# LargeWorldModel/LWM

Hardware: AMD Instinct MI355X
Metric: tokens/sec fwd+bwd, LWM-7B RingAttention hot path (32 layers x 32 heads x 128) (higher is better)
Workload: dtype bf16 (f32 logits/softmax/accumulate)

## Files before the change

lwm_amd/csrc/attn_bwd64.h:

```cpp
#pragma once

namespace lwm {

constexpr int kD4BK = 128;
constexpr int kD4BQ = 64;
constexpr int kD4Threads = 256;
constexpr int kD4Slots = 4;
constexpr int kD4TileBytes = kD4BQ * kRowBytes;
constexpr int kD4SlotBytes = 2 * kD4TileBytes;
constexpr int kD4OffStat = kD4Slots * kD4SlotBytes;
constexpr int kD4StatBytes = 3 * kD4BQ * 4;
constexpr int kD4LdsBytes = kD4OffStat + kD4Slots * kD4StatBytes;
#ifndef LWM_D4_AHEAD
#define LWM_D4_AHEAD 6
#endif
constexpr int kD4Ahead = LWM_D4_AHEAD;
static_assert(kD4Ahead >= 1 && kD4Ahead <= 7, "prefetch distance in fragments");
static_assert((kD4Ahead % 2) == 0, "paired requests need an even distance");

constexpr int q4_swz_of(int row) {
    const int r = row & 15;
    return (((r & 7) << 1) | (r >> 3)) ^ ((r >= 4 && r < 12) ? 1 : 0);
}
LWM_DEVICE int q4_swz(int row) { return q4_swz_of(row); }
LWM_DEVICE uint32_t q4_tile_off(int row, int slot) { return (uint32_t)(row * kRowBytes + ((slot ^ q4_swz(row)) << 4)); }
constexpr bool q4_image_ok() {
    for (int s = 0; s < 4; ++s)
        for (int grp = 0; grp < 4; ++grp) {
            unsigned long long banks = 0;
            for (int l = 0; l < 64; ++l) {
                const int m = l & 31;
                const bool first = m < 4 || (m >= 12 && m < 16) || (m >= 20 && m < 28);
                if (2 * (l >> 5) + (first ? 0 : 1) != grp) continue;
                const int slot = (4 * s + (l >> 4)) ^ q4_swz_of(l & 15);
                const unsigned long long b = 0xFull << (4 * slot);
                if (banks & b) return false;
                banks |= b;
            }
            if (banks != ~0ull) return false;
        }
    for (int db = 0; db < 8; ++db)
        for (int up = 0; up < 2; ++up)
            for (int half = 0; half < 2; ++half) {
                unsigned long long banks = 0;
                for (int l = 32 * half; l < 32 * half + 32; ++l) {
                    const int g = l >> 4, t = l & 15, row = 16 * up + 4 * g + (t >> 2);
                    const int slot = (2 * db + ((t & 3) >> 1)) ^ q4_swz_of(row);
                    const unsigned long long b = 0x3ull << (4 * slot + 2 * (t & 1));
                    if (banks & b) return false;
                    banks |= b;
                }
                if (banks != ~0ull) return false;
            }
    return true;
}
static_assert(q4_image_ok(), "a read of the Q | dO (K | V) image is bank-conflicted");

#ifdef LWM_EMU
LWM_DEVICE f32x4 mfma_16x16x32(bf16x8 a, bf16x8 b, f32x4 c) {
    emu::Wave& w = emu::g_blk->waves[emu::g_lane->tid >> 6];
    const int l = emu::g_lane->tid & 63;
    w.a[l] = a;
    w.b[l] = b;
    emu::wave_sync();
    f32x4 d;
    const int col = l & 15, g = l >> 4;
    for (int j = 0; j < 4; ++j) {
        const int row = 4 * g + j;
        float s = c[j];
        for (int k = 0; k < 32; ++k) s += (float)w.a[(k >> 3) * 16 + row][k & 7] * (float)w.b[(k >> 3) * 16 + col][k & 7];
        d[j] = s;
    }
    emu::wave_sync();
    return d;
}
LWM_DEVICE void q4_mfma_first(f32x4& d, bf16x8 a, bf16x8 b) { d = mfma_16x16x32(a, b, f32x4{0.0f, 0.0f, 0.0f, 0.0f}); }
LWM_DEVICE void q4_mfma(f32x4& d, bf16x8 a, bf16x8 b) { d = mfma_16x16x32(a, b, d); }
LWM_DEVICE void q4_mfma_c_first(f32x4& d, bf16x8 a, bf16x8 b, const f32x4& c) { d = mfma_16x16x32(a, b, c); }
LWM_DEVICE void q4_mfma_o(f32x4& d, bf16x8 a, bf16x8 b) { d = mfma_16x16x32(a, b, d); }
LWM_DEVICE void q4_mfma_o_first(f32x4& d, bf16x8 a, bf16x8 b) { d = mfma_16x16x32(a, b, f32x4{0.0f, 0.0f, 0.0f, 0.0f}); }
LWM_DEVICE void q4_opaque(f32x4 (&)[2]) {}
LWM_DEVICE void q4_settle_t(f32x4 (&)[4]) {}
LWM_DEVICE void q4_settle_acc(f32x4 (&)[16]) {}
#else
LWM_DEVICE void q4_mfma_first(f32x4& d, bf16x8 a, bf16x8 b) {
    asm volatile("v_mfma_f32_16x16x32_bf16 %0, %1, %2, 0" : "=&v"(d) : "v"(a), "a"(b));
}
LWM_DEVICE void q4_mfma(f32x4& d, bf16x8 a, bf16x8 b) {
    asm volatile("v_mfma_f32_16x16x32_bf16 %0, %1, %2, %0" : "+v"(d) : "v"(a), "a"(b));
}
LWM_DEVICE void q4_mfma_c_first(f32x4& d, bf16x8 a, bf16x8 b, const f32x4& c) {
    asm volatile("s_nop 1\n\tv_mfma_f32_16x16x32_bf16 %0, %1, %2, %3" : "=&v"(d) : "v"(a), "a"(b), "v"(c));
}
LWM_DEVICE void q4_mfma_o(f32x4& d, bf16x8 a, bf16x8 b) {
    asm volatile("v_mfma_f32_16x16x32_bf16 %0, %1, %2, %0" : "+a"(d) : "v"(a), "v"(b));
}
LWM_DEVICE void q4_mfma_o_first(f32x4& d, bf16x8 a, bf16x8 b) {
    asm volatile("v_mfma_f32_16x16x32_bf16 %0, %1, %2, 0" : "=&a"(d) : "v"(a), "v"(b));
}
LWM_DEVICE void q4_opaque(f32x4 (&x)[2]) { asm volatile("" : "+v"(x[0]), "+v"(x[1])); }
LWM_DEVICE void q4_settle_t(f32x4 (&s)[4]) { asm volatile("s_nop 7\n\ts_nop 7" : "+v"(s[0]), "+v"(s[1]), "+v"(s[2]), "+v"(s[3])); }
LWM_DEVICE void q4_settle_acc(f32x4 (&a)[16]) {
    asm volatile("s_nop 7\n\ts_nop 7"
                 : "+a"(a[0]), "+a"(a[1]), "+a"(a[2]), "+a"(a[3]), "+a"(a[4]), "+a"(a[5]), "+a"(a[6]), "+a"(a[7]), "+a"(a[8]),
                   "+a"(a[9]), "+a"(a[10]), "+a"(a[11]), "+a"(a[12]), "+a"(a[13]), "+a"(a[14]), "+a"(a[15]));
}
#endif

constexpr int kDsTileBytes = kD4BQ * 32 * 2;
constexpr int64_t ds_diag(int causal, int64_t q_start, int64_t k_start) {
    const int64_t lim = (int64_t)1 << 30, e = (k_start - q_start) >> 6;
    return !causal ? -lim : (e < -lim ? -lim : (e > lim ? lim : e));
}
constexpr int64_t ds_first_step(int64_t e, int64_t nst, int64_t kbi) {
    const int64_t s = e + 2 * kbi;
    return s < 0 ? 0 : (s > nst ? nst : s);
}
constexpr int64_t ds_steps_before(int64_t e, int64_t nst, int64_t kbi) {
    const int64_t jl = e >= 0 ? 0 : (1 - e) >> 1;
    const int64_t jh0 = e >= nst ? 0 : (nst - e + 1) >> 1;
    const int64_t jh = jh0 > jl ? jh0 : jl;
    const int64_t a = kbi < jl ? kbi : jl, b = kbi < jh ? kbi : jh;
    return kbi * nst - ((b - a) * e + (b - a) * (a + b - 1) + (kbi - b) * nst);
}
constexpr bool ds_geom_ok() {
    const int64_t es[] = {-(1 << 30), -1000, -9, -8, -3, -2, -1, 0, 1, 2, 3, 7, 8, 9, 40, 1 << 30};
    const int64_t ns[] = {1, 2, 3, 4, 6, 8, 9, 32};
    for (int64_t e : es)
        for (int64_t nst : ns) {
            int64_t sum = 0;
            for (int64_t kbi = 0; kbi < 24; ++kbi) {
                if (ds_steps_before(e, nst, kbi) != sum) return false;
                sum += nst - ds_first_step(e, nst, kbi);
            }
        }
    return true;
}
static_assert(ds_geom_ok(), "closed form of the workspace row offsets disagrees with the sum it stands for");
constexpr int64_t ds_wave_steps(int64_t e, int64_t nst, int64_t nkb, int64_t s) {
    if (s >= nst) return 0;
    const int64_t kend = s - e < 0 ? 0 : ((s - e) >> 1) + 1;
    return 4 * (kend < nkb ? kend : nkb);
}
constexpr int64_t ds_ws_bytes(int64_t B, int64_t H, int64_t Sq, int64_t Sk, int causal, int64_t q_start, int64_t k_start) {
    return B * H * ds_steps_before(ds_diag(causal, q_start, k_start), Sq / kD4BQ, Sk / kD4BK) * 4 * kDsTileBytes;
}

struct D4Ds {
    char* p;
    uint32_t v;
};
#ifdef LWM_EMU
LWM_DEVICE char* ds_uniform_ptr(char* p) { return p; }
template <int OFF>
LWM_DEVICE void d4_ds_store(const D4Ds& sw, bf16x8 x) { memcpy(sw.p + OFF + sw.v, &x, 16); }
#else
LWM_DEVICE char* ds_uniform_ptr(char* p) {
    const uint64_t a = (uint64_t)p;
    return (char*)(((uint64_t)(uint32_t)__builtin_amdgcn_readfirstlane((int)(a >> 32)) << 32) | (uint32_t)__builtin_amdgcn_readfirstlane((int)a));
}
template <int OFF>
LWM_DEVICE void d4_ds_store(const D4Ds& sw, bf16x8 x) {
    static_assert(OFF >= -4096 && OFF <= 4095, "13-bit signed instruction offset");
    asm volatile("global_store_dwordx4 %0, %1, %2 offset:%3 nt" ::"v"(sw.v), "v"(x), "s"(sw.p), "n"(OFF) : "memory");
}
#endif

struct D4Ctx {
    uint32_t qa[4];
    uint32_t tlo[8];
    uint32_t plo[8];
    uint32_t stat;
    float c;
};

#ifdef LWM_EMU
LWM_DEVICE float d4_mul(float a, float b) { return a * b; }
LWM_DEVICE void d4_dma_b32(uint32_t voff, const char* src, lds_t dst) { glds_load_b32(src + voff, dst); }
LWM_DEVICE void d4_settle_acc4(f32x16 (&)[4]) {}
#else
LWM_DEVICE float d4_mul(float a, float b) {
    float y;
    asm volatile("v_mul_f32 %0, %1, %2" : "=v"(y) : "v"(a), "v"(b));
    return y;
}
LWM_DEVICE void d4_dma_b32(uint32_t voff, const char* src, lds_t dst) {
    const uint64_t a = (uint64_t)src;
    const uint64_t u = ((uint64_t)(uint32_t)__builtin_amdgcn_readfirstlane((int)(a >> 32)) << 32) |
                       (uint32_t)__builtin_amdgcn_readfirstlane((int)a);
    asm volatile("s_mov_b32 m0, %2\n\ts_nop 0\n\tglobal_load_lds_dword %0, %1" ::"v"(voff), "s"(u), "s"(dst) : "memory");
}
LWM_DEVICE void d4_settle_acc4(f32x16 (&a)[4]) { asm volatile("s_nop 7\n\ts_nop 7" : "+a"(a[0]), "+a"(a[1]), "+a"(a[2]), "+a"(a[3])); }
#endif
LWM_DEVICE void d4_mfma_p_first(f32x4& d, bf16x8 a, bf16x8 b, const f32x4& c) { q4_mfma_c_first(d, a, b, c); }
LWM_DEVICE void d4_mfma_o_first(f32x4& d, bf16x8 a, bf16x8 b) { q4_mfma_o_first(d, a, b); }
LWM_DEVICE void d4_settle_t(f32x4 (&s)[4]) { q4_settle_t(s); }
LWM_DEVICE void d4_settle_acc(f32x4 (&dk)[16], f32x4 (&dv)[16]) {
    q4_settle_acc(dk);
    q4_settle_acc(dv);
}

LWM_DEVICE void d4_stage_offsets(const AttnParams& p, int wave, int lane, int st, uint32_t (&vq)[4], uint32_t (&vdo)[4]) {
    const int slot = lane & 15;
    for (int j = 0; j < 4; ++j) {
        const int row = 4 * (wave + 4 * j) + (lane >> 4);
        int qrow = st * kD4BQ + row;
        qrow = qrow < p.Sq ? qrow : p.Sq - 1;
        const int rel = qrow - st * kD4BQ;
        const int col = (slot ^ q4_swz(row)) << 3;
        vq[j] = (uint32_t)(((int64_t)rel * p.q_ss + col) * 2);
        vdo[j] = (uint32_t)(((int64_t)rel * p.do_ss + col) * 2);
    }
}

template <int HALF>
LWM_DEVICE bf16x8 d4_frag(const D4Ctx& cx, int f) {
    if (f >= 32) {
        const int g = f - 32;
        return lds_read_b128(cx.qa[g >> 2] + ((g >> 1) & 1) * kD4TileBytes + (g & 1) * 16 * kRowBytes + (HALF == 0 ? 32 * kRowBytes : 0));
    }
    if (f < 16) return lds_read_b128(cx.qa[f >> 2] + ((f >> 1) & 1) * kD4TileBytes + (f & 1) * 16 * kRowBytes + HALF * 32 * kRowBytes);
    const int j = f - 16, db = 2 * (j >> 2) + (j & 1);
    const uint32_t a = (HALF == 0 ? cx.plo[db] : cx.tlo[db]) + (HALF == 0 ? 32 * kRowBytes : 0) + (((j >> 1) & 1) ? 0 : kD4TileBytes);
    bf16x4 lo = lds_read_tr16(a);
    bf16x4 up = lds_read_tr16(a + 16 * kRowBytes);
    bf16x8 o;
    o[0] = lo[0]; o[1] = lo[1]; o[2] = lo[2]; o[3] = lo[3];
    o[4] = up[0]; o[5] = up[1]; o[6] = up[2]; o[7] = up[3];
    return o;
}

struct D4Sched {
    int F[16], E[16], M[16], P[8], D[8], W[2];
};
constexpr bool d4_sched_ok(const D4Sched& c) {
    int load[64] = {};
    for (int e = 0; e < 16; ++e) {
        if (c.F[e] < 3 || c.F[e] > 31 || c.E[e] <= c.F[e] || c.M[e] <= c.E[e] || c.M[e] > 61) return false;
        load[c.F[e]] += 1;
        load[c.E[e]] += 2;
        load[c.M[e]] += 1;
    }
    for (int i = 0; i < 8; ++i) {
        if (c.P[i] < 32 || c.P[i] > 61 || c.P[i] <= c.E[2 * i] || c.P[i] <= c.E[2 * i + 1]) return false;
        if (c.D[i] < 32 || c.D[i] > 61 || c.D[i] <= c.M[2 * i] || c.D[i] <= c.M[2 * i + 1]) return false;
        load[c.P[i]] += 1;
        load[c.D[i]] += 1;
    }
    for (int h = 0; h < 2; ++h) {
        if (c.W[h] != 63) return false;
        for (int i = 4 * h; i < 4 * h + 4; ++i)
            if (c.W[h] <= c.D[i]) return false;
    }
    for (int g = 0; g < 64; ++g)
        if (load[g] > 2) return false;
    return true;
}
constexpr D4Sched kD4Sched = {
     {3, 3, 4, 4, 5, 5, 6, 6, 7, 7, 8, 8, 9, 9, 10, 10},
     {11, 12, 13, 14, 15, 16, 17, 18, 19, 20, 21, 22, 23, 24, 25, 26},
     {27, 27, 28, 28, 29, 29, 30, 30, 31, 31, 32, 32, 33, 33, 34, 34},
     {35, 35, 36, 36, 37, 37, 38, 38},
     {39, 39, 40, 40, 41, 41, 42, 42},
     {63, 63}};
static_assert(d4_sched_ok(kD4Sched), "filler schedule violates a dependency or the issue budget of a gap");

struct D4Dma {
    const char* q_src;
    const char* do_src;
    lds_t dst;
};

struct D4Regs {
    f32x4 s[4];
    f32x4 dp[2][4];
    f32x4 ndl[2];
    float nl[8];
    float t[16];
    float ds[16];
    bf16x8 pb[2], dsb[2];
    uint32_t pw[8], dw[8];
    bf16x8 fr[8];
};

template <int G, int PAR>
LWM_DEVICE void d4_fillers(const D4Ctx& cx, D4Regs& rg) {
#pragma unroll
    for (int e = 0; e < 16; ++e) {
        if (kD4Sched.F[e] == G) rg.t[e] = f4_fma(rg.s[e >> 2][e & 3], cx.c, rg.nl[4 * ((e >> 2) & 1) + (e & 3)]);
        if (kD4Sched.E[e] == G) rg.t[e] = f4_exp2(rg.t[e]);
        if (kD4Sched.M[e] == G) rg.ds[e] = d4_mul(rg.t[e], rg.dp[PAR][e >> 2][e & 3]);
    }
#pragma unroll
    for (int i = 0; i < 8; ++i) {
        if (kD4Sched.P[i] == G) rg.pw[i] = f4_cvt_pk(rg.t[2 * i], rg.t[2 * i + 1]);
        if (kD4Sched.D[i] == G) rg.dw[i] = f4_cvt_pk(rg.ds[2 * i], rg.ds[2 * i + 1]);
    }
#pragma unroll
    for (int h = 0; h < 2; ++h) {
        int lp = 0, ld = 0;
        for (int i = 4 * h; i < 4 * h + 4; ++i) {
            lp = kD4Sched.P[i] > lp ? kD4Sched.P[i] : lp;
            ld = kD4Sched.D[i] > ld ? kD4Sched.D[i] : ld;
        }
        if (lp == G) rg.pb[h] = __builtin_bit_cast(bf16x8, u32x4{rg.pw[4 * h], rg.pw[4 * h + 1], rg.pw[4 * h + 2], rg.pw[4 * h + 3]});
        if (ld == G) rg.dsb[h] = __builtin_bit_cast(bf16x8, u32x4{rg.dw[4 * h], rg.dw[4 * h + 1], rg.dw[4 * h + 2], rg.dw[4 * h + 3]});
    }
}

template <int G, int BASE>
LWM_DEVICE void d4_ds_stores(const D4Ds& sw, const D4Regs& rg) {
    if constexpr (kD4Sched.W[0] == G) d4_ds_store<BASE>(sw, rg.dsb[0]);
    if constexpr (kD4Sched.W[1] == G) d4_ds_store<BASE + 1024>(sw, rg.dsb[1]);
}

template <int HALF, bool HAS_PREV, bool DMA, bool DS, int M = 0>
LWM_DEVICE void d4_x(const D4Ctx& cx, D4Regs& rg, const bf16x8 (&kf)[8], const bf16x8 (&vf)[8], const uint32_t (&vq)[4],
                     const uint32_t (&vdo)[4], const D4Dma& dm, const D4Ds& sw) {
    if constexpr (M < 32) {
        if constexpr ((M & 3) == 0) {
            constexpr int f0 = (M >> 1) + kD4Ahead;
            rg.fr[f0 & 7] = d4_frag<HALF>(cx, f0);
            sched_fence();
            rg.fr[(f0 + 1) & 7] = d4_frag<HALF>(cx, f0 + 1);
        }
        if constexpr (M == 10 || M == 18) {
            constexpr int qh = M == 18 ? 1 : 0;
            const f32x4 v = lds_read_f32x4(cx.stat + (HALF * 32 + 16 * qh) * 4);
            rg.nl[4 * qh + 0] = v[0]; rg.nl[4 * qh + 1] = v[1]; rg.nl[4 * qh + 2] = v[2]; rg.nl[4 * qh + 3] = v[3];
        }
        sched_fence();
        {
            constexpr int f = (M >> 1) ^ 1, qh = f & 1, kh = ((M >> 1) ^ M) & 1;
            constexpr int s = f >> 2, t = 2 * kh + qh;
            if constexpr (((f >> 1) & 1) == 0) {
                if constexpr (s == 0) q4_mfma_first(rg.s[t], rg.fr[f & 7], kf[4 * kh]);
                else q4_mfma(rg.s[t], rg.fr[f & 7], kf[4 * kh + s]);
            } else {
                if constexpr (s == 0) d4_mfma_p_first(rg.dp[HALF][t], rg.fr[f & 7], vf[4 * kh], rg.ndl[qh]);
                else q4_mfma(rg.dp[HALF][t], rg.fr[f & 7], vf[4 * kh + s]);
            }
        }
        if constexpr (DMA && (M & 3) == 3) {
            constexpr int i = M >> 2, j = i >> 1;
            if constexpr ((i & 1) == 0) f4_dma1(vq[j], dm.q_src, dm.dst + 4096 * j);
            else f4_dma1(vdo[j], dm.do_src, dm.dst + kD4TileBytes + 4096 * j);
        }
        if constexpr (HAS_PREV) d4_fillers<32 + M, HALF ^ 1>(cx, rg);
        if constexpr (HAS_PREV && DS) d4_ds_stores<32 + M, HALF == 1 ? -kDsTileBytes : kDsTileBytes / 2>(sw, rg);
        sched_fence();
        d4_x<HALF, HAS_PREV, DMA, DS, M + 1>(cx, rg, kf, vf, vq, vdo, dm, sw);
    }
}

template <int HALF, bool HAS_META>
LWM_DEVICE void d4_mask(const D4Ctx& cx, f32x4 (&s)[4], const int (&rel)[2], const int32_t (&kseg)[2]) {
#pragma unroll
    for (int qh = 0; qh < 2; ++qh) {
        u32x4 sg = {0u, 0u, 0u, 0u};
        if (HAS_META) sg = lds_read_u32x4(cx.stat + 2 * kD4BQ * 4 + HALF * 32 * 4 + 16 * qh * 4);
#pragma unroll
        for (int kh = 0; kh < 2; ++kh)
#pragma unroll
            for (int j = 0; j < 4; ++j) {
                const bool vis = (!HAS_META || (int32_t)sg[j] == kseg[kh]) && (16 * qh + j >= rel[kh]);
                s[2 * kh + qh][j] = vis ? s[2 * kh + qh][j] : -INFINITY;
            }
    }
}

template <int HALF, bool HAS_PREV, bool NEXT, bool INIT, int J = 0>
LWM_DEVICE void d4_y(const D4Ctx& cx, D4Regs& rg, f32x4 (&dk)[16], f32x4 (&dv)[16], uint32_t statn) {
    if constexpr (J < 32) {
        if constexpr ((J & 3) == 0 && (16 + (J >> 1) + kD4Ahead < 32 || NEXT)) {
            constexpr int f0 = 16 + (J >> 1) + kD4Ahead;
            rg.fr[f0 & 7] = d4_frag<HALF>(cx, f0);
            sched_fence();
            rg.fr[(f0 + 1) & 7] = d4_frag<HALF>(cx, f0 + 1);
        }
        if constexpr (NEXT && (J == 22 || J == 26)) {
            constexpr int qh = J == 26 ? 1 : 0;
            rg.ndl[qh] = lds_read_f32x4(statn + kD4BQ * 4 + ((HALF ^ 1) * 32 + 16 * qh) * 4);
        }
        sched_fence();
        if constexpr (HAS_PREV) {
            constexpr int jf = (J >> 1) ^ 1, kh = ((J >> 1) ^ J) & 1;
            constexpr int db = 2 * (jf >> 2) + (jf & 1);
            if constexpr (((jf >> 1) & 1) == 0) {
                if constexpr (INIT) d4_mfma_o_first(dv[2 * db + kh], rg.fr[(16 + jf) & 7], rg.pb[kh]);
                else q4_mfma_o(dv[2 * db + kh], rg.fr[(16 + jf) & 7], rg.pb[kh]);
            } else {
                if constexpr (INIT) d4_mfma_o_first(dk[2 * db + kh], rg.fr[(16 + jf) & 7], rg.dsb[kh]);
                else q4_mfma_o(dk[2 * db + kh], rg.fr[(16 + jf) & 7], rg.dsb[kh]);
            }
        }
        d4_fillers<J, HALF>(cx, rg);
        sched_fence();
        d4_y<HALF, HAS_PREV, NEXT, INIT, J + 1>(cx, rg, dk, dv, statn);
    }
}

template <int PAR, bool DS, int G = 32>
LWM_DEVICE void d4_drain_fill(const D4Ctx& cx, D4Regs& rg, const D4Ds& sw) {
    if constexpr (G < 64) {
        d4_fillers<G, PAR>(cx, rg);
        if constexpr (DS) d4_ds_stores<G, kDsTileBytes / 2>(sw, rg);
        d4_drain_fill<PAR, DS, G + 1>(cx, rg, sw);
    }
}
template <int H, int J = 0>
LWM_DEVICE void d4_drain_mfma(D4Regs& rg, f32x4 (&dk)[16], f32x4 (&dv)[16]) {
    if constexpr (J < 16) {
        constexpr int jf = 8 * H + (J >> 1), kh = ((J >> 1) ^ J) & 1;
        constexpr int db = 2 * (jf >> 2) + (jf & 1);
        if constexpr (((jf >> 1) & 1) == 0) q4_mfma_o(dv[2 * db + kh], rg.fr[jf & 7], rg.pb[kh]);
        else q4_mfma_o(dk[2 * db + kh], rg.fr[jf & 7], rg.dsb[kh]);
        d4_drain_mfma<H, J + 1>(rg, dk, dv);
    }
}
template <int PAR, bool DS>
LWM_DEVICE void d4_drain(const D4Ctx& cx, D4Regs& rg, f32x4 (&dk)[16], f32x4 (&dv)[16], const D4Ds& sw) {
    d4_drain_fill<PAR, DS>(cx, rg, sw);
#pragma unroll
    for (int j = 0; j < 8; ++j) rg.fr[j] = d4_frag<0>(cx, 16 + j);
    sched_fence();
    d4_drain_mfma<0>(rg, dk, dv);
    sched_fence();
#pragma unroll
    for (int j = 0; j < 8; ++j) rg.fr[j] = d4_frag<0>(cx, 24 + j);
    sched_fence();
    d4_drain_mfma<1>(rg, dk, dv);
    sched_fence();
}

LWM_DEVICE void d4_epi_tile_write(lds_t tb, const f32x4 (&acc)[16], float scale, int c, int g) {
#pragma unroll
    for (int db = 0; db < 8; ++db)
#pragma unroll
        for (int kh = 0; kh < 2; ++kh) {
            const f32x4 a = acc[2 * db + kh];
            lds_write_f32x4(tb + (uint32_t)((16 * kh + c) * kEpiRowBytes + (16 * db + 4 * g) * 4),
                            f32x4{a[0] * scale, a[1] * scale, a[2] * scale, a[3] * scale});
        }
}

LWM_DEVICE void d4_store_tiles(const AttnParams& p, lds_t tb, const f32x4 (&dk)[16], const f32x4 (&dv)[16], int b, int h,
                               int row0, int lane) {
    const int l31 = lane & 31, hi = lane >> 5, col = l31 * 4;
    const int Sk = p.Sk;
    const bool carry = p.carry_in != 0, fin = p.final_out != 0;
    const int rows = Sk - (row0 + hi);
    const int64_t acc0 = ((((int64_t)b * Sk + row0 + hi) * p.H + h) * kHeadDim + col) * 4;
    const int64_t acc_step = (int64_t)2 * p.H * kHeadDim * 4;
#pragma unroll
    for (int which = 0; which < 2; ++which) {
        if (which) wave_lds_fence();
        d4_epi_tile_write(tb, which ? dv : dk, which ? 1.0f : p.scale, lane & 15, lane >> 4);
        wave_lds_fence();
        char* ap = (char*)(which ? p.dv_acc : p.dk_acc) + acc0;
        const int64_t o_ss = which ? p.dv_ss : p.dk_ss;
        char* op = (char*)((which ? p.dv : p.dk) + (int64_t)b * (which ? p.dv_sb : p.dk_sb) + (int64_t)(row0 + hi) * o_ss +
                           (int64_t)h * (which ? p.dv_sh : p.dk_sh) + col);
        const int64_t out_step = 2 * o_ss * 2;
        if (fin && !carry) {
#pragma unroll
            for (int i = 0; i < 16; ++i) {
                const f32x4 x = epi_tile_read(tb, i, lane);
                if (2 * i < rows) global_store_b64(op + i * out_step, u32x2{pack_bf16x2(x[0], x[1]), pack_bf16x2(x[2], x[3])});
            }
        } else if (!fin && !carry) {
#pragma unroll
            for (int i = 0; i < 16; ++i) {
                const f32x4 x = epi_tile_read(tb, i, lane);
                if (2 * i < rows) global_store_f32x4((float*)(ap + i * acc_step), x);
            }
        } else {
#pragma unroll
            for (int i = 0; i < 16; ++i) {
                f32x4 x = epi_tile_read(tb, i, lane);
                if (2 * i < rows) {
                    const f32x4 c = global_load_f32x4((const float*)(ap + i * acc_step));
                    x[0] += c[0]; x[1] += c[1]; x[2] += c[2]; x[3] += c[3];
                    if (fin) global_store_b64(op + i * out_step, u32x2{pack_bf16x2(x[0], x[1]), pack_bf16x2(x[2], x[3])});
                    else global_store_f32x4((float*)(ap + i * acc_step), x);
                }
            }
        }
    }
}

template <bool HAS_META, bool DS = false>
LWM_DEVICE void attn_bwd_dkdv4_body(const AttnParams& p) {
    static_assert(!(HAS_META && DS), "the hand-over has no key meta");
#ifdef LWM_PROF
    const unsigned long long d4_entry = __builtin_amdgcn_s_memtime();
    unsigned long long d4_head = 0, d4_epi = 0;
#endif
    const lds_t lds = dyn_lds();
    const int tid = thread_idx();
    const int wave = wave_uniform(tid >> 6), lane = tid & 63, l15 = lane & 15, g4 = lane >> 4;

    const int nkb = (p.Sk + kD4BK - 1) / kD4BK;
    const int HB = p.H * p.B;
    int lin = block_idx_x(), kbi, hb;
    if ((HB & 7) == 0) {
        int xcd = lin & 7, i = lin >> 3;
        hb = xcd + 8 * (i / nkb);
        kbi = i % nkb;
    } else {
        hb = lin / nkb;
        kbi = lin % nkb;
    }
    const int b = hb / p.H, h = hb % p.H;
    const bf16_t* qb = p.q + (int64_t)b * p.q_sb + (int64_t)h * p.q_sh;
    const bf16_t* kb = p.k + (int64_t)b * p.k_sb + (int64_t)h * p.k_sh;
    const bf16_t* vb = p.v + (int64_t)b * p.v_sb + (int64_t)h * p.v_sh;
    const bf16_t* dob = p.dout + (int64_t)b * p.do_sb + (int64_t)h * p.do_sh;

    int k_row[2], kr[2];
    bool k_ok[2];
#pragma unroll
    for (int kh = 0; kh < 2; ++kh) {
        k_row[kh] = kbi * kD4BK + wave * 32 + 16 * kh + l15;
        k_ok[kh] = k_row[kh] < p.Sk;
        kr[kh] = k_ok[kh] ? k_row[kh] : p.Sk - 1;
    }
    bf16x8 kf[8], vf[8];
#pragma unroll
    for (int i = 0; i < 8; ++i) kf[i] = f4_load_agpr(kb + (int64_t)kr[i >> 2] * p.k_ss + 32 * (i & 3) + 8 * g4);
#pragma unroll
    for (int i = 0; i < 8; ++i) vf[i] = f4_load_agpr(vb + (int64_t)kr[i >> 2] * p.v_ss + 32 * (i & 3) + 8 * g4);
    const PosMap qm = q_map(p);
    const PosTab qt_ = load_postab(qm);
    const int64_t k_base = pos_base(load_postab(k_map(p)), kbi * kD4BK);
    int32_t kseg[2] = {0, 0};
    if (HAS_META) {
#pragma unroll
        for (int kh = 0; kh < 2; ++kh) {
            kseg[kh] = kSegInvalid;
            if (k_ok[kh]) {
                const bool valid = p.key_valid ? (p.key_valid[(int64_t)b * p.Sk + k_row[kh]] != 0) : true;
                if (valid) kseg[kh] = p.seg_k ? p.seg_k[(int64_t)b * p.Sk + k_row[kh]] : 0;
            }
        }
    }

    int nst = (p.Sq + kD4BQ - 1) / kD4BQ;
    int st0 = 0;
    if (p.causal) st0 = tiles_below(qt_, kD4BQ, nst, k_base + (int64_t)kbi * kD4BK - 1);
    if (HAS_META && p.segb_q && p.segb_k && st0 < nst) {
        const int nbq = (p.Sq + 31) >> 5, nbk = (p.Sk + 31) >> 5;
        int smin, smax, lo, hi2;
        seg_own_range(p.segb_k + (int64_t)b * nbk * 2, nbk, kbi * (kD4BK / 32), kD4BK / 32, smin, smax);
        seg_narrow<kD4Threads>(p.segb_q + (int64_t)b * nbq * 2, nbq, kD4BQ / 32, st0, nst, smin, smax, lds + kD4OffStat, tid, lo, hi2);
        st0 = lo;
        nst = hi2;
    }
    const int n = nst > st0 ? nst - st0 : 0;

    f32x4 dk[16], dv[16];
    if (n == 0)
#pragma unroll
        for (int i = 0; i < 16; ++i) {
            dk[i] = f32x4{0.0f, 0.0f, 0.0f, 0.0f};
            dv[i] = f32x4{0.0f, 0.0f, 0.0f, 0.0f};
        }
    if (n == 0) {
        f4_load_agpr_wait8(kf);
        f4_load_agpr_wait8(vf);
    }

    if (n > 0) {
        D4Ctx cx;
        cx.c = p.scale * kLog2e;
#pragma unroll
        for (int s = 0; s < 4; ++s) cx.qa[s] = lds + q4_tile_off(l15, 4 * s + g4);
#pragma unroll
        for (int db = 0; db < 8; ++db) {
            cx.tlo[db] = lds + q4_tile_off(4 * g4 + (l15 >> 2), 2 * db + ((l15 & 3) >> 1)) + (l15 & 1) * 8;
            cx.plo[db] = cx.tlo[db];
        }
        cx.stat = lds + kD4OffStat + 16 * g4;

        const int64_t q_step_bytes = (int64_t)kD4BQ * p.q_ss * 2, do_step_bytes = (int64_t)kD4BQ * p.do_ss * 2;
        uint32_t vq[4], vdo[4];
        d4_stage_offsets(p, wave, lane, 0, vq, vdo);
        const int64_t Sqp = bwd_stat_pad(p.Sq);
        const char* stat_src = (const char*)(p.delta + bwd_stat_row((int64_t)b * p.H + h, Sqp) + (wave == 1 ? Sqp : 0));
        bool stat_on = wave < 2;
        if (HAS_META && wave == 2 && p.seg_q) {
            stat_src = (const char*)(p.seg_q + (int64_t)b * p.Sq);
            stat_on = true;
        }
        const lds_t stat_dst = lds + kD4OffStat + (uint32_t)(wave < 3 ? wave : 0) * kD4BQ * 4;
        const uint32_t vstat = (uint32_t)lane * 4;
        if (HAS_META && !p.seg_q)
            for (int sl = 0; sl < kD4Slots; ++sl)
                if (tid < kD4BQ) lds_write_i32(lds + kD4OffStat + sl * kD4StatBytes + 2 * kD4BQ * 4 + tid * 4, 0);
        auto stage_step = [&](int i) {
            const int st = nst - 1 - i;
            const lds_t dst = lds + (i & 3) * kD4SlotBytes + (uint32_t)wave * 1024;
            const char* qs = (const char*)qb + st * q_step_bytes;
            const char* ds = (const char*)dob + st * do_step_bytes;
            if (stat_on) {
                int row = st * kD4BQ + lane;
                if (HAS_META && wave == 2) row = row < p.Sq ? row : p.Sq - 1;
                glds_load_b32(stat_src + (int64_t)row * 4, stat_dst + (i & 3) * kD4StatBytes);
            }
            if (st * kD4BQ + kD4BQ > p.Sq) {
                uint32_t v2[4], d2[4];
                d4_stage_offsets(p, wave, lane, st, v2, d2);
                f4_dma<4>(v2, qs, dst);
                f4_dma<4>(d2, ds, dst + kD4TileBytes);
            } else {
                f4_dma<4>(vq, qs, dst);
                f4_dma<4>(vdo, ds, dst + kD4TileBytes);
            }
        };

        stage_step(0);
        if (n > 1) stage_step(1);
        f4_load_agpr_wait8(kf);
        f4_load_agpr_wait8(vf);
        block_sync();

        auto clamp32 = [](int64_t x) -> int { return x > (1 << 30) ? (1 << 30) : (x < -(1 << 30) ? -(1 << 30) : (int)x); };
        int k_rel[2];
#pragma unroll
        for (int kh = 0; kh < 2; ++kh) k_rel[kh] = clamp32(k_base + k_row[kh] - p.q_start) - 4 * g4;
        PosCursor qc = cursor_begin(qt_);
        auto q_rel_of = [&](int ub) -> int {
            cursor_seek(qm, qc, ub);
            return clamp32(qc.base + ub - p.q_start);
        };
        const int mask_end = p.causal ? 32 * tiles_reaching(qt_, 32, (p.Sq + 31) / 32, k_base + (int64_t)kbi * kD4BK + wave * 32 + 31 - 1) : 0;
        auto needs_causal = [&](int ub) -> bool { return ub < mask_end; };
        const int32_t own_seg = wave_uniform(kseg[0]);
        const bool own_uniform = HAS_META && !wave_any(kseg[0] != own_seg || kseg[1] != own_seg || own_seg == kSegInvalid);
        auto rel_of = [&](int ub, int (&rel)[2]) {
            if (!p.causal) {
                rel[0] = rel[1] = -64;
                return;
            }
            const int qr = q_rel_of(ub);
#pragma unroll
            for (int kh = 0; kh < 2; ++kh) {
                const int64_t d = (int64_t)k_rel[kh] - qr;
                rel[kh] = d > 64 ? 64 : (d < -64 ? -64 : (int)d);
            }
        };

        D4Regs rg;
#pragma unroll
        for (int t = 0; t < 4; ++t) {
            rg.s[t] = f32x4{0.0f, 0.0f, 0.0f, 0.0f};
            rg.dp[0][t] = f32x4{0.0f, 0.0f, 0.0f, 0.0f};
            rg.dp[1][t] = f32x4{0.0f, 0.0f, 0.0f, 0.0f};
        }
#pragma unroll
        for (int r = 0; r < 16; ++r) {
            rg.t[r] = 0.0f;
            rg.ds[r] = 0.0f;
        }
#pragma unroll
        for (int r = 0; r < 8; ++r) rg.nl[r] = 0.0f;
#pragma unroll
        for (int t = 0; t < 2; ++t) {
            rg.pb[t] = zero_bf16x8();
            rg.dsb[t] = zero_bf16x8();
        }
#pragma unroll
        for (int j = 0; j < 8; ++j) rg.fr[j] = zero_bf16x8();
        D4Dma dm = {};
        D4Ds sw = {};
        if (DS) {
            const int64_t e = ds_diag(p.causal, p.q_start, p.k_start);
            const int64_t tile = ((int64_t)hb * ds_steps_before(e, nst, nkb) + ds_steps_before(e, nst, kbi)) * 4 + (int64_t)wave * n + (n - 1);
            sw.p = ds_uniform_ptr(p.ds_ws + (tile + 1) * kDsTileBytes);
            sw.v = (uint32_t)lane * 16;
        }
#pragma unroll
        for (int j = 0; j < kD4Ahead; ++j) rg.fr[j] = d4_frag<0>(cx, j);
#pragma unroll
        for (int qh = 0; qh < 2; ++qh) rg.ndl[qh] = lds_read_f32x4(cx.stat + kD4BQ * 4 + 16 * qh * 4);

#define LWM_D4_MASK(HALF_, HAS_PREV_, ub_)                                                                          \
    do {                                                                                                            \
         \
         \
        if (!(HAS_PREV_)) d4_settle_t(rg.s);         \
        if ((HAS_META && !uni_) || needs_causal(ub_)) {                                                             \
            if (HAS_PREV_) d4_settle_t(rg.s);                                                                       \
            int rel_[2];                                                                                            \
            rel_of(ub_, rel_);                                                                                      \
            if (HAS_META && !uni_) d4_mask<HALF_, HAS_META>(cx, rg.s, rel_, kseg);                                  \
            else d4_mask<HALF_, false>(cx, rg.s, rel_, kseg);                                                       \
        }                                                                                                           \
    } while (0)
#ifdef LWM_PROF
        unsigned long long d4p[12] = {0, 0, 0, 0, 0, 0, 0, 0, 0, 0, 0, 0}, d4t = __builtin_amdgcn_s_memtime();
        const unsigned long long d4t0 = d4t;
        d4_head = d4t - d4_entry;
#define D4_LAP(slot)                                                  \
    do {                                                              \
        const unsigned long long now_ = __builtin_amdgcn_s_memtime(); \
        d4p[slot] += now_ - d4t;                                      \
        d4t = now_;                                                   \
    } while (0)
#if LWM_PROF > 1
#define D4_LAP2(slot) D4_LAP(slot)
#else
#define D4_LAP2(slot)
#endif
#else
#define D4_LAP(slot)
#define D4_LAP2(slot)
#endif
        int ub = (nst - 1) * kD4BQ;
        const char* q_src2 = (const char*)qb + (int64_t)(nst - 3) * q_step_bytes;
        const char* do_src2 = (const char*)dob + (int64_t)(nst - 3) * do_step_bytes;
        const char* st_src2 = stat_src + (int64_t)(nst - 3) * kD4BQ * 4;
#define LWM_D4_STEP(i, FIRST, PIPE)                                                                                 \
    do {                                                                                                            \
        if (PIPE) {                                                                                                 \
            if (stat_on) d4_dma_b32(vstat, st_src2, stat_dst + (((i) + 2) & 3) * kD4StatBytes);                     \
            dm.q_src = q_src2;                                                                                      \
            dm.do_src = do_src2;                                                                                    \
            dm.dst = lds + (((i) + 2) & 3) * kD4SlotBytes + (uint32_t)wave * 1024;                                  \
            q_src2 -= q_step_bytes;                                                                                 \
            do_src2 -= do_step_bytes;                                                                               \
            st_src2 -= kD4BQ * 4;                                                                                   \
        }                                                                                                           \
        const uint32_t d_ = (((i) & 3) == 3) ? (uint32_t)(-3 * kD4SlotBytes) : (uint32_t)kD4SlotBytes;             \
        const uint32_t e_ = (((i) & 3) == 3) ? (uint32_t)(-3 * kD4StatBytes) : (uint32_t)kD4StatBytes;             \
        const int32_t segw_ = HAS_META ? seg_step_word(cx.stat - 16 * g4 + 2 * kD4BQ * 4, lane) : 0;                \
        d4_x<0, !(FIRST), PIPE, DS>(cx, rg, kf, vf, vq, vdo, dm, sw);                                                       \
        const bool uni_ = HAS_META && seg_step_uniform(segw_, own_uniform, own_seg);                                \
        D4_LAP2(0);                                                                                                 \
        LWM_D4_MASK(0, !(FIRST), ub);                                                                               \
        D4_LAP2(1);                                                                                                 \
        d4_y<0, !(FIRST), true, false>(cx, rg, dk, dv, cx.stat);                                                    \
        D4_LAP2(2);                                                                                                 \
        d4_x<1, true, false, DS>(cx, rg, kf, vf, vq, vdo, dm, sw);                                                  \
        for (int s_ = 0; s_ < 4; ++s_) cx.qa[s_] += d_;                                                             \
        D4_LAP2(3);                                                                                                 \
        LWM_D4_MASK(1, true, ub + 32);                                                                              \
        D4_LAP2(4);                                                                                                 \
        d4_y<1, true, true, FIRST>(cx, rg, dk, dv, cx.stat + e_);                                                   \
        D4_LAP(5);                                                                                                  \
        ub -= kD4BQ;                                                                                                \
          \
          \
        if ((FIRST) || !(PIPE)) d4_settle_acc(dk, dv);                                                              \
          \
          \
          \
        if (DS) {                                                                                                   \
            if (FIRST) wait_vmem_le<2>();                                                                           \
            else wait_vmem_le<4>();                                                                                 \
            sw.p -= kDsTileBytes;                                                                                   \
        } else {                                                                                                    \
            glds_wait_all();                                                                                        \
        }                                                                                                           \
        D4_LAP(6);                                                                                                  \
        block_sync_lds();                                                                                           \
        D4_LAP(7);                                                                                                  \
        for (int db_ = 0; db_ < 8; ++db_) {                                                                         \
            cx.plo[db_] = cx.tlo[db_];                                                                              \
            cx.tlo[db_] += d_;                                                                                      \
        }                                                                                                           \
        cx.stat += e_;                                                                                              \
        D4_LAP(8);                                                                                                  \
    } while (0)

        int i = 0;
        if (n > 2) {
            LWM_D4_STEP(0, true, true);
#ifdef LWM_PROF
            for (int j = 0; j < 12; ++j) d4p[j] = 0;
            d4t = __builtin_amdgcn_s_memtime();
#endif
            for (i = 1; i + 2 < n; ++i) {
                LWM_D4_STEP(i, false, true);
#ifdef LWM_PROF
                d4p[9] += 1;
#endif
            }
#ifdef LWM_PROF
            if (!HAS_META && hb == 0 && kbi == 0 && lane == 0 && p.out_acc) {
                d4p[10] = __builtin_amdgcn_s_memtime() - d4t0;
                for (int j = 0; j < 11; ++j) ((unsigned long long*)p.out_acc)[wave * 16 + j] = d4p[j];
            }
#endif
            for (; i < n; ++i) LWM_D4_STEP(i, false, false);
        } else {
            LWM_D4_STEP(0, true, false);
            if (n > 1) LWM_D4_STEP(1, false, false);
        }
#undef LWM_D4_STEP
#undef D4_LAP
#undef D4_LAP2
#undef LWM_D4_MASK
        d4_drain<1, DS>(cx, rg, dk, dv, sw);
        d4_settle_acc(dk, dv);
    }

    d4_settle_acc(dk, dv);
#ifdef LWM_PROF
    d4_epi = __builtin_amdgcn_s_memtime() - d4_entry;
#endif
    if (DS) glds_wait_all();
    block_sync_lds();
    d4_store_tiles(p, lds + (uint32_t)wave * kEpiTileBytes, dk, dv, b, h, kbi * kD4BK + wave * 32, lane);
#ifdef LWM_PROF
    if (!HAS_META && hb == 0 && kbi == 0 && lane == 0 && p.out_acc) {
        asm volatile("s_waitcnt vmcnt(0)" ::: "memory");
        unsigned long long* o_ = (unsigned long long*)p.out_acc + wave * 16;
        o_[11] = __builtin_amdgcn_s_memtime() - d4_entry;
        o_[12] = d4_head;
        o_[13] = d4_epi;
    }
#endif
}


LWM_KERNEL(kD4Threads) void attn_bwd_dkdv4_kernel(AttnParams p) { attn_bwd_dkdv4_body<false>(p); }
LWM_KERNEL(kD4Threads) void attn_bwd_dkdv4_meta_kernel(AttnParams p) { attn_bwd_dkdv4_body<true>(p); }
LWM_KERNEL(kD4Threads) void attn_bwd_dkdv4_ds_kernel(AttnParams p) { attn_bwd_dkdv4_body<false, true>(p); }


constexpr int kQ4BQ = 128;
constexpr int kQ4BK = 64;
constexpr int kQ4OffMeta = kD4Slots * kD4SlotBytes;
constexpr int kQ4LdsBytes = kQ4OffMeta + kD4Slots * kQ4BK * 4;


struct Q4Sched {
    int F[16], E[16], M[16], D[8];
};
constexpr bool q4_sched_ok(const Q4Sched& c) {
    int load[48] = {};
    for (int e = 0; e < 16; ++e) {
        if (c.F[e] < 3 || c.E[e] <= c.F[e] || c.M[e] <= c.E[e] || c.M[e] > 45) return false;
        load[c.F[e]] += 1;
        load[c.E[e]] += 2;
        load[c.M[e]] += 1;
    }
    for (int i = 0; i < 8; ++i) {
        if (c.D[i] < 16 || c.D[i] > 45 || c.D[i] <= c.M[2 * i] || c.D[i] <= c.M[2 * i + 1]) return false;
        load[c.D[i]] += 1;
    }
    for (int g = 0; g < 48; ++g)
        if (load[g] > 2) return false;
    return true;
}
constexpr Q4Sched kQ4Sched = {
     {3, 4, 5, 6, 7, 8, 9, 10, 11, 12, 13, 13, 14, 14, 15, 15},
     {16, 17, 18, 19, 20, 21, 22, 23, 24, 25, 26, 27, 28, 29, 30, 31},
     {32, 32, 33, 33, 34, 34, 35, 35, 36, 36, 37, 37, 38, 38, 39, 39},
     {40, 40, 41, 41, 42, 42, 43, 43}};
static_assert(q4_sched_ok(kQ4Sched), "filler schedule violates a dependency or the issue budget of a gap");

struct Q4Ctx {
    uint32_t ka[4];
    uint32_t tlo[8];
    uint32_t plo[8];
    uint32_t meta;
    float c, nl[2];
};

struct Q4Regs {
    f32x4 s[2][4], dp[2][4];
    f32x4 ndl[2];
    float t[16], ds[16];
    bf16x8 dsb[2];
    uint32_t dw[8];
    bf16x8 fr[8];
};


template <int HALF>
LWM_DEVICE bf16x8 q4_frag(const Q4Ctx& cx, int f) {
    if (f >= 24) {
        const int g = f - 24;
        return lds_read_b128(cx.ka[g >> 2] + (g & 1) * kD4TileBytes + ((g >> 1) & 1) * 16 * kRowBytes + (HALF == 0 ? 32 * kRowBytes : 0));
    }
    if (f < 16) return lds_read_b128(cx.ka[f >> 2] + (f & 1) * kD4TileBytes + ((f >> 1) & 1) * 16 * kRowBytes + HALF * 32 * kRowBytes);
    const int db = f - 16;
    const uint32_t a = (HALF == 0 ? cx.plo[db] : cx.tlo[db]) + (HALF == 0 ? 32 * kRowBytes : 0);
    bf16x4 lo = lds_read_tr16(a);
    bf16x4 up = lds_read_tr16(a + 16 * kRowBytes);
    bf16x8 o;
    o[0] = lo[0]; o[1] = lo[1]; o[2] = lo[2]; o[3] = lo[3];
    o[4] = up[0]; o[5] = up[1]; o[6] = up[2]; o[7] = up[3];
    return o;
}

template <int G, int PAR>
LWM_DEVICE void q4_fillers(const Q4Ctx& cx, Q4Regs& rg) {
#pragma unroll
    for (int e = 0; e < 16; ++e) {
        if (kQ4Sched.F[e] == G) rg.t[e] = f4_fma(rg.s[PAR][e >> 2][e & 3], cx.c, cx.nl[e >> 3]);
        if (kQ4Sched.E[e] == G) rg.t[e] = f4_exp2(rg.t[e]);
        if (kQ4Sched.M[e] == G) rg.ds[e] = d4_mul(rg.t[e], rg.dp[PAR][e >> 2][e & 3]);
    }
#pragma unroll
    for (int i = 0; i < 8; ++i)
        if (kQ4Sched.D[i] == G) rg.dw[i] = f4_cvt_pk(rg.ds[2 * i], rg.ds[2 * i + 1]);
#pragma unroll
    for (int h = 0; h < 2; ++h) {
        int ld = 0;
        for (int i = 4 * h; i < 4 * h + 4; ++i) ld = kQ4Sched.D[i] > ld ? kQ4Sched.D[i] : ld;
        if (ld == G) rg.dsb[h] = __builtin_bit_cast(bf16x8, u32x4{rg.dw[4 * h], rg.dw[4 * h + 1], rg.dw[4 * h + 2], rg.dw[4 * h + 3]});
    }
}
template <int HALF, bool HAS_PREV, bool DMA, int M = 0>
LWM_DEVICE void q4_x(const Q4Ctx& cx, Q4Regs& rg, const bf16x8 (&qf)[8], const bf16x8 (&dof)[8], const uint32_t (&vk)[4],
                     const uint32_t (&vv)[4], const D4Dma& dm) {
    if constexpr (M < 32) {
        if constexpr ((M & 3) == 0) {
            constexpr int f0 = (M >> 1) + kD4Ahead;
            rg.fr[f0 & 7] = q4_frag<HALF>(cx, f0);
            sched_fence();
            rg.fr[(f0 + 1) & 7] = q4_frag<HALF>(cx, f0 + 1);
        }
        sched_fence();
        {
            constexpr int f = (M >> 1) ^ 1, qh = M & 1;
            constexpr int s = f >> 2, t = 2 * qh + ((f >> 1) & 1);
            if constexpr ((f & 1) == 0) {
                if constexpr (s == 0) q4_mfma_first(rg.s[HALF][t], rg.fr[f & 7], qf[4 * qh]);
                else q4_mfma(rg.s[HALF][t], rg.fr[f & 7], qf[4 * qh + s]);
            } else {
                if constexpr (s == 0) q4_mfma_c_first(rg.dp[HALF][t], rg.fr[f & 7], dof[4 * qh], rg.ndl[qh]);
                else q4_mfma(rg.dp[HALF][t], rg.fr[f & 7], dof[4 * qh + s]);
            }
        }
        if constexpr (DMA && (M & 3) == 3) {
            constexpr int i = M >> 2, j = i >> 1;
            if constexpr ((i & 1) == 0) f4_dma1(vk[j], dm.q_src, dm.dst + 4096 * j);
            else f4_dma1(vv[j], dm.do_src, dm.dst + kD4TileBytes + 4096 * j);
        }
        if constexpr (HAS_PREV) q4_fillers<16 + M, HALF ^ 1>(cx, rg);
        sched_fence();
        q4_x<HALF, HAS_PREV, DMA, M + 1>(cx, rg, qf, dof, vk, vv, dm);
    }
}

template <int HALF, bool HAS_META>
LWM_DEVICE void q4_mask(const Q4Ctx& cx, f32x4 (&s)[4], const int (&rel)[2], const int32_t (&seg_q)[2]) {
#pragma unroll
    for (int kh = 0; kh < 2; ++kh) {
        u32x4 sg = {0u, 0u, 0u, 0u};
        if (HAS_META) sg = lds_read_u32x4(cx.meta + HALF * 32 * 4 + 16 * kh * 4);
#pragma unroll
        for (int qh = 0; qh < 2; ++qh)
#pragma unroll
            for (int j = 0; j < 4; ++j) {
                const bool vis = (!HAS_META || (int32_t)sg[j] == seg_q[qh]) && (16 * kh + j <= rel[qh]);
                s[2 * qh + kh][j] = vis ? s[2 * qh + kh][j] : -INFINITY;
            }
    }
}

template <int HALF, bool HAS_PREV, bool INIT, int J = 0>
LWM_DEVICE void q4_y(const Q4Ctx& cx, Q4Regs& rg, f32x4 (&dq)[16]) {
    if constexpr (J < 16) {
        if constexpr ((J & 3) == 0) {
            constexpr int f0 = 16 + (J >> 1) + kD4Ahead;
            rg.fr[f0 & 7] = q4_frag<HALF>(cx, f0);
            sched_fence();
            rg.fr[(f0 + 1) & 7] = q4_frag<HALF>(cx, f0 + 1);
        }
        sched_fence();
        if constexpr (HAS_PREV) {
            constexpr int db = (J >> 1) ^ 1, qh = J & 1;
            if constexpr (INIT) q4_mfma_o_first(dq[2 * db + qh], rg.fr[(16 + db) & 7], rg.dsb[qh]);
            else q4_mfma_o(dq[2 * db + qh], rg.fr[(16 + db) & 7], rg.dsb[qh]);
        }
        q4_fillers<J, HALF>(cx, rg);
        sched_fence();
        q4_y<HALF, HAS_PREV, INIT, J + 1>(cx, rg, dq);
    }
}

template <int PAR, int G = 16>
LWM_DEVICE void q4_drain_fill(const Q4Ctx& cx, Q4Regs& rg) {
    if constexpr (G < 48) {
        q4_fillers<G, PAR>(cx, rg);
        q4_drain_fill<PAR, G + 1>(cx, rg);
    }
}
template <int J = 0>
LWM_DEVICE void q4_drain_mfma(Q4Regs& rg, f32x4 (&dq)[16]) {
    if constexpr (J < 16) {
        q4_mfma_o(dq[J], rg.fr[J >> 1], rg.dsb[J & 1]);
        q4_drain_mfma<J + 1>(rg, dq);
    }
}
template <int PAR>
LWM_DEVICE void q4_drain(const Q4Ctx& cx, Q4Regs& rg, f32x4 (&dq)[16]) {
    q4_drain_fill<PAR>(cx, rg);
#pragma unroll
    for (int j = 0; j < 8; ++j) rg.fr[j] = q4_frag<0>(cx, 16 + j);
    sched_fence();
    q4_drain_mfma(rg, dq);
}

LWM_DEVICE void q4_stage_offsets(const AttnParams& p, int wave, int lane, int st, uint32_t (&vk)[4], uint32_t (&vv)[4]) {
    const int slot = lane & 15;
    for (int j = 0; j < 4; ++j) {
        const int row = 4 * (wave + 4 * j) + (lane >> 4);
        int krow = st * kQ4BK + row;
        krow = krow < p.Sk ? krow : p.Sk - 1;
        const int rel = krow - st * kQ4BK;
        const int col = (slot ^ q4_swz(row)) << 3;
        vk[j] = (uint32_t)(((int64_t)rel * p.k_ss + col) * 2);
        vv[j] = (uint32_t)(((int64_t)rel * p.v_ss + col) * 2);
    }
}

template <int QH>
LWM_DEVICE void q4_store(const AttnParams& p, const f32x4 (&dq)[16], int b, int h, int q_row, int g4) {
    const bool carry = p.carry_in != 0, fin = p.final_out != 0;
    const float sc = p.scale;
    bf16_t* const op = p.dq + (int64_t)b * p.dq_sb + (int64_t)q_row * p.dq_ss + (int64_t)h * p.dq_sh + 4 * g4;
    float* const ap = p.dq_acc + (int64_t)b * p.dqa_sb + (int64_t)q_row * p.dqa_ss + (int64_t)h * p.dqa_sh + 4 * g4;
    if (fin && !carry) {
#pragma unroll
        for (int db = 0; db < 8; ++db) {
            const f32x4 a = dq[2 * db + QH];
            global_store_b64(op + 16 * db, u32x2{pack_bf16x2(a[0] * sc, a[1] * sc), pack_bf16x2(a[2] * sc, a[3] * sc)});
        }
    } else {
#pragma unroll
        for (int db = 0; db < 8; ++db) {
            const f32x4 a = dq[2 * db + QH];
            float o0 = a[0] * sc, o1 = a[1] * sc, o2 = a[2] * sc, o3 = a[3] * sc;
            if (carry) {
                const f32x4 c = global_load_f32x4(ap + 16 * db);
                o0 += c[0]; o1 += c[1]; o2 += c[2]; o3 += c[3];
            }
            if (fin) global_store_b64(op + 16 * db, u32x2{pack_bf16x2(o0, o1), pack_bf16x2(o2, o3)});
            else global_store_f32x4(ap + 16 * db, f32x4{o0, o1, o2, o3});
        }
    }
}

template <bool HAS_META>
LWM_DEVICE void attn_bwd_dq4_body(const AttnParams& p) {
    const lds_t lds = dyn_lds();
    const int tid = thread_idx();
    const int wave = wave_uniform(tid >> 6), lane = tid & 63, l15 = lane & 15, g4 = lane >> 4;

    const int nqb = (p.Sq + kQ4BQ - 1) / kQ4BQ;
    const int HB = p.H * p.B;
    int lin = block_idx_x(), qbi, hb;
    if ((HB & 7) == 0) {
        int xcd = lin & 7, i = lin >> 3;
        hb = xcd + 8 * (i / nqb);
        qbi = nqb - 1 - (i % nqb);
    } else {
        hb = lin / nqb;
        qbi = nqb - 1 - (lin % nqb);
    }
    const int b = hb / p.H, h = hb % p.H;
    const bf16_t* qb = p.q + (int64_t)b * p.q_sb + (int64_t)h * p.q_sh;
    const bf16_t* kb = p.k + (int64_t)b * p.k_sb + (int64_t)h * p.k_sh;
    const bf16_t* vb = p.v + (int64_t)b * p.v_sb + (int64_t)h * p.v_sh;
// ... 397 lines not shown
```

Measured before the change: 33000.

## Move per-step vmem wait and barrier before the second dK/dV update

Moves the per-step vmem wait and LDS barrier from the end of the step to before the second d4_y half. The wait now uses a compile-time count of the loads the step itself issued, so those loads can stay in flight while d4_y runs. To make that count the same on every wave, all waves now issue the stat DMA, with odd waves loading the second delta row. This trades a few redundant stat loads for a barrier placed earlier and overlapped with the accumulation work, and it relies on the hand-derived count matching the real issue order.

Result: no change. 33320, median of 6 (+1.0%).

```diff
diff --git a/lwm_amd/csrc/attn_bwd64.h b/lwm_amd/csrc/attn_bwd64.h
--- a/lwm_amd/csrc/attn_bwd64.h
+++ b/lwm_amd/csrc/attn_bwd64.h
@@ -264,6 +264,19 @@
      {39, 39, 40, 40, 41, 41, 42, 42},
      {63, 63}};
 static_assert(d4_sched_ok(kD4Sched), "filler schedule violates a dependency or the issue budget of a gap");
+constexpr int d4_own_vmem(bool PIPE, bool FIRST, bool DS) {
+    int n = PIPE ? 1 : 0;
+    for (int m = 0; m < 32; ++m) n += PIPE && (m & 3) == 3 ? 1 : 0;
+    for (int half = 0; half < 2; ++half)
+        for (int m = 0; m < 32; ++m)
+            for (int h = 0; h < 2; ++h) n += DS && !(FIRST && half == 0) && kD4Sched.W[h] == 32 + m ? 1 : 0;
+    return n;
+}
+static_assert(d4_own_vmem(true, false, true) == 1 + 8 + 4 && d4_own_vmem(true, true, true) == 1 + 8 + 2 &&
+                  d4_own_vmem(false, false, true) == 4 && d4_own_vmem(true, false, false) == 1 + 8 &&
+                  d4_own_vmem(false, true, false) == 0,
+              "the counted wait of a step does not count what the step issues");
+static_assert(d4_own_vmem(true, false, true) < 64, "vmcnt is a 6-bit counter");
 
 struct D4Dma {
     const char* q_src;
@@ -586,13 +599,10 @@
         uint32_t vq[4], vdo[4];
         d4_stage_offsets(p, wave, lane, 0, vq, vdo);
         const int64_t Sqp = bwd_stat_pad(p.Sq);
-        const char* stat_src = (const char*)(p.delta + bwd_stat_row((int64_t)b * p.H + h, Sqp) + (wave == 1 ? Sqp : 0));
-        bool stat_on = wave < 2;
-        if (HAS_META && wave == 2 && p.seg_q) {
-            stat_src = (const char*)(p.seg_q + (int64_t)b * p.Sq);
-            stat_on = true;
-        }
-        const lds_t stat_dst = lds + kD4OffStat + (uint32_t)(wave < 3 ? wave : 0) * kD4BQ * 4;
+        const bool stat_seg = HAS_META && wave == 2 && p.seg_q;
+        const char* stat_src = stat_seg ? (const char*)(p.seg_q + (int64_t)b * p.Sq)
+                                        : (const char*)(p.delta + bwd_stat_row((int64_t)b * p.H + h, Sqp) + ((wave & 1) ? Sqp : 0));
+        const lds_t stat_dst = lds + kD4OffStat + (uint32_t)(stat_seg ? 2 : (wave & 1)) * kD4BQ * 4;
         const uint32_t vstat = (uint32_t)lane * 4;
         if (HAS_META && !p.seg_q)
             for (int sl = 0; sl < kD4Slots; ++sl)
@@ -602,11 +612,9 @@
             const lds_t dst = lds + (i & 3) * kD4SlotBytes + (uint32_t)wave * 1024;
             const char* qs = (const char*)qb + st * q_step_bytes;
             const char* ds = (const char*)dob + st * do_step_bytes;
-            if (stat_on) {
-                int row = st * kD4BQ + lane;
-                if (HAS_META && wave == 2) row = row < p.Sq ? row : p.Sq - 1;
-                glds_load_b32(stat_src + (int64_t)row * 4, stat_dst + (i & 3) * kD4StatBytes);
-            }
+            int row = st * kD4BQ + lane;
+            if (stat_seg) row = row < p.Sq ? row : p.Sq - 1;
+            glds_load_b32(stat_src + (int64_t)row * 4, stat_dst + (i & 3) * kD4StatBytes);
             if (st * kD4BQ + kD4BQ > p.Sq) {
                 uint32_t v2[4], d2[4];
                 d4_stage_offsets(p, wave, lane, st, v2, d2);
@@ -723,7 +731,7 @@
 #define LWM_D4_STEP(i, FIRST, PIPE)                                                                                 \
     do {                                                                                                            \
         if (PIPE) {                                                                                                 \
-            if (stat_on) d4_dma_b32(vstat, st_src2, stat_dst + (((i) + 2) & 3) * kD4StatBytes);                     \
+            d4_dma_b32(vstat, st_src2, stat_dst + (((i) + 2) & 3) * kD4StatBytes);                                  \
             dm.q_src = q_src2;                                                                                      \
             dm.do_src = do_src2;                                                                                    \
             dm.dst = lds + (((i) + 2) & 3) * kD4SlotBytes + (uint32_t)wave * 1024;                                  \
@@ -745,26 +753,19 @@
         for (int s_ = 0; s_ < 4; ++s_) cx.qa[s_] += d_;                                                             \
         D4_LAP2(3);                                                                                                 \
         LWM_D4_MASK(1, true, ub + 32);                                                                              \
-        D4_LAP2(4);                                                                                                 \
+        D4_LAP(4);                                                                                                  \
+            \
+        wait_vmem_le<d4_own_vmem(PIPE, FIRST, DS)>();                                                               \
+        D4_LAP(6);                                                                                                  \
+        block_sync_lds();                                                                                           \
+        D4_LAP(7);                                                                                                  \
         d4_y<1, true, true, FIRST>(cx, rg, dk, dv, cx.stat + e_);                                                   \
         D4_LAP(5);                                                                                                  \
         ub -= kD4BQ;                                                                                                \
           \
           \
         if ((FIRST) || !(PIPE)) d4_settle_acc(dk, dv);                                                              \
-          \
-          \
-          \
-        if (DS) {                                                                                                   \
-            if (FIRST) wait_vmem_le<2>();                                                                           \
-            else wait_vmem_le<4>();                                                                                 \
-            sw.p -= kDsTileBytes;                                                                                   \
-        } else {                                                                                                    \
-            glds_wait_all();                                                                                        \
-        }                                                                                                           \
-        D4_LAP(6);                                                                                                  \
-        block_sync_lds();                                                                                           \
-        D4_LAP(7);                                                                                                  \
+        if (DS) sw.p -= kDsTileBytes;                                                                               \
         for (int db_ = 0; db_ < 8; ++db_) {                                                                         \
             cx.plo[db_] = cx.tlo[db_];                                                                              \
             cx.tlo[db_] += d_;                                                                                      \
```
